# andrewendlinger/xmris

Measured on AMD Instinct MI355X. Metric: spectra/sec (zero_fill->apodize->FFT->autophase), n_time=4096; HBM-roofline %, higher is better.
Workload: dtype f32

## Files before the change

### xmris_amd/csrc/xm_coarse.h

```cpp
#pragma once
#include "xm_kernels.h"

typedef _Float16 xm_h8 __attribute__((ext_vector_type(8)));
typedef _Float16 xm_h2 __attribute__((ext_vector_type(2)));
typedef float xm_f16v __attribute__((ext_vector_type(16)));

struct CoarseArgs {
  const void* in;
  const float* window;
  const Cx<float>* w1024;
  float* est;
  unsigned long long* gkey;
  long long in_stride;
  long long n_batch;
  float scale2;
};

constexpr int kCoarseWaves = 4;

XM_DEV Cx<float> coarse_w1024(const Cx<float>* __restrict__ t, unsigned k) {
  k &= 1023u;
  const Cx<float> w = t[k & 511u];
  return (k & 512u) ? mk<float>(-w.re, -w.im) : w;
}

XM_DEV xm_h8 coarse_pack(const float* v) {
  union {
    xm_h8 v8;
    xm_h2 v2[4];
  } u;
#pragma unroll
  for (int j = 0; j < 4; ++j) {
    const xm_f2 p = {v[2 * j], v[2 * j + 1]};
    u.v2[j] = __builtin_convertvector(p, xm_h2);
  }
  return u.v8;
}

template <bool IN64>
__global__ __launch_bounds__(64 * kCoarseWaves, 2) void k_coarse_mfma(CoarseArgs A) {
  const unsigned lane = threadIdx.x & 63u, r = lane & 31u, h = lane >> 5;
  const long long wave = (long long)blockIdx.x * kCoarseWaves + (threadIdx.x >> 6);
  const long long n_waves = (long long)gridDim.x * kCoarseWaves;

  xm_h8 b1r, b1i, b1n, a2r[2], a2i[2], a2n[2];
  {
    float cr[8], ci[8], cn[8];
#pragma unroll
    for (int j = 0; j < 8; ++j) {
      const Cx<float> w = coarse_w1024(A.w1024, 32u * ((8u * h + (unsigned)j) * r));
      cr[j] = w.re;
      ci[j] = w.im;
      cn[j] = -w.im;
    }
    b1r = coarse_pack(cr);
    b1i = coarse_pack(ci);
    b1n = coarse_pack(cn);
#pragma unroll
    for (int s = 0; s < 2; ++s) {
#pragma unroll
      for (int j = 0; j < 8; ++j) {
        const unsigned n2 = 16u * s + 8u * ((unsigned)j >> 2) + 4u * h + ((unsigned)j & 3u);
        const Cx<float> w = coarse_w1024(A.w1024, 32u * (n2 * r));
        cr[j] = w.re;
        ci[j] = w.im;
        cn[j] = -w.im;
      }
      a2r[s] = coarse_pack(cr);
      a2i[s] = coarse_pack(ci);
      a2n[s] = coarse_pack(cn);
    }
  }
  float twr[16], twi[16];
#pragma unroll
  for (int q = 0; q < 16; ++q) {
    const unsigned n2 = ((unsigned)q & 3u) + 8u * ((unsigned)q >> 2) + 4u * h;
    const Cx<float> w = coarse_w1024(A.w1024, n2 * r);
    twr[q] = w.re;
    twi[q] = w.im;
  }
  float wnd[8];
#pragma unroll
  for (int j = 0; j < 8; ++j) wnd[j] = A.window[32u * (8u * h + (unsigned)j) + r];

  auto fetch = [&](long long s, Cx<float>* x) {
    if constexpr (IN64) {
      const xm_d2* __restrict__ row = reinterpret_cast<const xm_d2*>(A.in) + s * A.in_stride;
#pragma unroll
      for (int j = 0; j < 8; ++j) {
        const xm_d2 v = __builtin_nontemporal_load(row + 32u * (8u * h + (unsigned)j) + r);
        x[j] = mk<float>((float)v.x, (float)v.y);
      }
      return;
    }
    const xm_f2* __restrict__ row = reinterpret_cast<const xm_f2*>(A.in) + s * A.in_stride;
#pragma unroll
    for (int j = 0; j < 8; ++j) {
      const xm_f2 v = __builtin_nontemporal_load(row + 32u * (8u * h + (unsigned)j) + r);
      x[j] = mk<float>(v.x, v.y);
    }
  };

  unsigned best_key = 0u, best_row = 0u;
  bool have = false;
  constexpr int DEPTH = 1;
  Cx<float> nx[DEPTH][8];
  long long s = wave;
#pragma unroll
  for (int d = 0; d < DEPTH; ++d)
    if (s + d * n_waves < A.n_batch) fetch(s + d * n_waves, nx[d]);
  auto one_row = [&](Cx<float>* cur, long long s) {
    float re[8], im[8];
    float m = 0.f;
#pragma unroll
    for (int j = 0; j < 8; ++j) {
      re[j] = cur[j].re * wnd[j];
      im[j] = cur[j].im * wnd[j];
      m = fmaxf(m, fmaxf(fabsf(re[j]), fabsf(im[j])));
    }
    if (s + DEPTH * n_waves < A.n_batch) fetch(s + DEPTH * n_waves, cur);
    unsigned e = (wave_reduce_u32<true>(__float_as_uint(m)) >> 23) & 0xffu;
    e = e > 253u ? 253u : (e < 1u ? 1u : e);
    const float up = __uint_as_float((254u - e) << 23);
    const float down = __uint_as_float(e << 23);
#pragma unroll
    for (int j = 0; j < 8; ++j) {
      re[j] *= up;
      im[j] *= up;
    }
    const xm_h8 ar = coarse_pack(re), ai = coarse_pack(im);
    xm_f16v d1r = {0.f}, d1i = {0.f};
    d1r = __builtin_amdgcn_mfma_f32_32x32x16_f16(ar, b1r, d1r, 0, 0, 0);
    d1r = __builtin_amdgcn_mfma_f32_32x32x16_f16(ai, b1n, d1r, 0, 0, 0);
    d1i = __builtin_amdgcn_mfma_f32_32x32x16_f16(ar, b1i, d1i, 0, 0, 0);
    d1i = __builtin_amdgcn_mfma_f32_32x32x16_f16(ai, b1r, d1i, 0, 0, 0);
    float zr[16], zi[16];
#pragma unroll
    for (int q = 0; q < 16; ++q) {
      zr[q] = d1r[q] * twr[q] - d1i[q] * twi[q];
      zi[q] = d1r[q] * twi[q] + d1i[q] * twr[q];
    }
    xm_f16v d2r = {0.f}, d2i = {0.f};
#pragma unroll
    for (int k = 0; k < 2; ++k) {
      const xm_h8 br = coarse_pack(zr + 8 * k), bi = coarse_pack(zi + 8 * k);
      d2r = __builtin_amdgcn_mfma_f32_32x32x16_f16(a2r[k], br, d2r, 0, 0, 0);
      d2r = __builtin_amdgcn_mfma_f32_32x32x16_f16(a2n[k], bi, d2r, 0, 0, 0);
      d2i = __builtin_amdgcn_mfma_f32_32x32x16_f16(a2r[k], bi, d2i, 0, 0, 0);
      d2i = __builtin_amdgcn_mfma_f32_32x32x16_f16(a2i[k], br, d2i, 0, 0, 0);
    }
    float bv = -1.f;
#pragma unroll
    for (int q = 0; q < 16; ++q) bv = fmaxf(bv, d2r[q] * d2r[q] + d2i[q] * d2i[q]);
    bv = amax_nan_if_unset(bv);
    bv = bv * (down * down) * A.scale2;
    const unsigned key = wave_reduce_u32<true>(bv != bv ? 0x7fc00000u : __float_as_uint(bv));
    const unsigned row = (unsigned)s;
    const bool take = !have || key > best_key;
    best_key = take ? key : best_key;
    best_row = take ? row : best_row;
    have = true;
    if (lane == 0u) A.est[s] = __uint_as_float(key);
  };
  for (; s < A.n_batch; s += DEPTH * n_waves) {
#pragma unroll
    for (int d = 0; d < DEPTH; ++d)
      if (s + d * n_waves < A.n_batch) one_row(nx[d], s + d * n_waves);
  }
  if (A.gkey && have && lane == 0u)
    atomicMax(A.gkey + (blockIdx.x % XM_KEY_SLOTS) * XM_KEY_STRIDE,
              ((unsigned long long)best_key << 32) | (unsigned long long)(0xffffffffu - best_row));
}
```

Measured before the change: 58.88 million.

## Deepen coarse-kernel prefetch pipeline using buffer loads with branchless bounds

Raises the software prefetch depth of the coarse MFMA kernel from 1 to 3 rows for f32 input and 2 rows for f64 input, so more HBM loads are in flight per wave. Global loads become raw buffer loads whose resource size is zero for out-of-range rows, so out-of-range fetches return zero without per-row branches. Raw bits are kept in registers and converted only when used, and the wave index is made scalar with readfirstlane. The deeper pipeline costs more VGPRs, which could lower occupancy under the launch bounds of 2.

```diff
diff --git a/xmris_amd/csrc/xm_coarse.h b/xmris_amd/csrc/xm_coarse.h
--- a/xmris_amd/csrc/xm_coarse.h
+++ b/xmris_amd/csrc/xm_coarse.h
@@ -17,6 +17,7 @@
 };
 
 constexpr int kCoarseWaves = 4;
+constexpr int kCoarseDepth = 3, kCoarseDepth64 = 2;
 
 XM_DEV Cx<float> coarse_w1024(const Cx<float>* __restrict__ t, unsigned k) {
   k &= 1023u;
@@ -40,7 +41,7 @@
 template <bool IN64>
 __global__ __launch_bounds__(64 * kCoarseWaves, 2) void k_coarse_mfma(CoarseArgs A) {
   const unsigned lane = threadIdx.x & 63u, r = lane & 31u, h = lane >> 5;
-  const long long wave = (long long)blockIdx.x * kCoarseWaves + (threadIdx.x >> 6);
+  const long long wave = (long long)blockIdx.x * kCoarseWaves + __builtin_amdgcn_readfirstlane((int)(threadIdx.x >> 6));
   const long long n_waves = (long long)gridDim.x * kCoarseWaves;
 
   xm_h8 b1r, b1i, b1n, a2r[2], a2i[2], a2n[2];
@@ -83,42 +84,48 @@
 #pragma unroll
   for (int j = 0; j < 8; ++j) wnd[j] = A.window[32u * (8u * h + (unsigned)j) + r];
 
-  auto fetch = [&](long long s, Cx<float>* x) {
-    if constexpr (IN64) {
-      const xm_d2* __restrict__ row = reinterpret_cast<const xm_d2*>(A.in) + s * A.in_stride;
-#pragma unroll
-      for (int j = 0; j < 8; ++j) {
-        const xm_d2 v = __builtin_nontemporal_load(row + 32u * (8u * h + (unsigned)j) + r);
-        x[j] = mk<float>((float)v.x, (float)v.y);
-      }
-      return;
-    }
-    const xm_f2* __restrict__ row = reinterpret_cast<const xm_f2*>(A.in) + s * A.in_stride;
+  constexpr unsigned EB = IN64 ? 16u : 8u;
+  typedef unsigned raw_t __attribute__((ext_vector_type(IN64 ? 4 : 2)));
+  const unsigned voff = (256u * h + r) * EB;
+  auto fetch = [&](long long s, raw_t* x) {
+    const bool ok = s < A.n_batch;
+    const char* row = reinterpret_cast<const char*>(A.in) + (size_t)((ok ? s : 0) * A.in_stride) * EB;
+    const __amdgpu_buffer_rsrc_t rs = xm_rsrc(row, ok ? 512u * EB : 0u);
 #pragma unroll
     for (int j = 0; j < 8; ++j) {
-      const xm_f2 v = __builtin_nontemporal_load(row + 32u * (8u * h + (unsigned)j) + r);
-      x[j] = mk<float>(v.x, v.y);
+      if constexpr (IN64) x[j] = __builtin_amdgcn_raw_buffer_load_b128(rs, voff, 32u * EB * (unsigned)j, 2);
+      else x[j] = __builtin_amdgcn_raw_buffer_load_b64(rs, voff, 32u * EB * (unsigned)j, 2);
     }
   };
 
   unsigned best_key = 0u, best_row = 0u;
   bool have = false;
-  constexpr int DEPTH = 1;
-  Cx<float> nx[DEPTH][8];
+  constexpr int DEPTH = IN64 ? kCoarseDepth64 : kCoarseDepth;
+  raw_t nx[DEPTH][8];
   long long s = wave;
 #pragma unroll
-  for (int d = 0; d < DEPTH; ++d)
-    if (s + d * n_waves < A.n_batch) fetch(s + d * n_waves, nx[d]);
-  auto one_row = [&](Cx<float>* cur, long long s) {
+  for (int d = 0; d < DEPTH; ++d) {
+    fetch(s + d * n_waves, nx[d]);
+    __builtin_amdgcn_sched_barrier(0);
+  }
+  auto one_row = [&](raw_t* cur, long long s) {
     float re[8], im[8];
     float m = 0.f;
 #pragma unroll
     for (int j = 0; j < 8; ++j) {
-      re[j] = cur[j].re * wnd[j];
-      im[j] = cur[j].im * wnd[j];
+      if constexpr (IN64) {
+        double d[2];
+        __builtin_memcpy(d, &cur[j], 16);
+        re[j] = (float)d[0] * wnd[j];
+        im[j] = (float)d[1] * wnd[j];
+      } else {
+        re[j] = __uint_as_float(cur[j].x) * wnd[j];
+        im[j] = __uint_as_float(cur[j].y) * wnd[j];
+      }
       m = fmaxf(m, fmaxf(fabsf(re[j]), fabsf(im[j])));
     }
-    if (s + DEPTH * n_waves < A.n_batch) fetch(s + DEPTH * n_waves, cur);
+    fetch(s + DEPTH * n_waves, cur);
+    if (s >= A.n_batch) return;
     unsigned e = (wave_reduce_u32<true>(__float_as_uint(m)) >> 23) & 0xffu;
     e = e > 253u ? 253u : (e < 1u ? 1u : e);
     const float up = __uint_as_float((254u - e) << 23);
@@ -164,8 +171,7 @@
   };
   for (; s < A.n_batch; s += DEPTH * n_waves) {
 #pragma unroll
-    for (int d = 0; d < DEPTH; ++d)
-      if (s + d * n_waves < A.n_batch) one_row(nx[d], s + d * n_waves);
+    for (int d = 0; d < DEPTH; ++d) one_row(nx[d], s + d * n_waves);
   }
   if (A.gkey && have && lane == 0u)
     atomicMax(A.gkey + (blockIdx.x % XM_KEY_SLOTS) * XM_KEY_STRIDE,
```

After: 59.07 million (median of 6 runs). No clear change (+0.3%).
